# tlemane/kmtricks

Measured on AMD Instinct MI355X. Metric: k-mers merged/s (merge stage, sum over partitions of input records / time), higher is better.
Workload: dtype u64 keys / u32 counts (integer)

## Files before the change

### kmtricks_amd/csrc/kmx_api.hip

```cpp
#include "kmx_host.hpp"

#include <algorithm>
#include <chrono>
#include <cmath>
#include <sys/mman.h>
#include <unordered_map>
#include <mutex>
#include <cstdlib>
#include <cstring>
#include <memory>

using namespace kmx;

static thread_local std::string g_create_err;

void* kmx_ctx::dalloc(size_t bytes)
{
  if (bytes == 0) bytes = 256;
  if (bytes >= (8u << 20)) { size_t p2 = (size_t)1 << 23; while (p2 * 2 <= bytes) p2 *= 2; const size_t q = p2 >> 3; bytes = (bytes + q - 1) / q * q; }
  int best = -1;
  for (size_t i = 0; i < pool.size(); i++)
    if (!pool[i].used && pool[i].bytes >= bytes && pool[i].bytes <= 2 * bytes + (1u << 20) &&
        (best < 0 || pool[i].bytes < pool[best].bytes)) best = (int)i;
  if (best >= 0) { pool[best].used = true; return pool[best].p; }
// ... 511 lines not shown
    KMX_HIP(ctx, launch_merge_bf(mode == KMX_MODE_BFC, d_tasks, d_items, R->n_items, d_ticket, R->grid, R->bf_lds, ctx->stream));
  } else if (R->use_cols) {
    const TaskDev* d_subs = reinterpret_cast<const TaskDev*>(R->d_meta + R->o_subtasks);
    const uint2* d_subitems = reinterpret_cast<const uint2*>(R->d_meta + R->o_subitems);
    const ColsDev* d_cols = reinterpret_cast<const ColsDev*>(R->d_meta + R->o_cols);
    const uint2* d_citems = reinterpret_cast<const uint2*>(R->d_meta + R->o_citems);
    static const bool overlap = getenv("KMX_COLS_PREP_OVERLAP") != nullptr;
    hipStream_t ps = overlap ? ctx->aux : ctx->stream;
    if (!R->ev_pre) KMX_HIP(ctx, hipEventCreateWithFlags(&R->ev_pre, hipEventDisableTiming));
    if (overlap && ctx->stream_shared) {
      KMX_HIP(ctx, hipEventRecord(R->ev_pre, ctx->stream));
      KMX_HIP(ctx, hipStreamWaitEvent(ctx->aux, R->ev_pre, 0));
    }
    if (!overlap) KMX_HIP(ctx, hipStreamWaitEvent(ctx->stream, R->ev_up, 0));
    KMX_HIP(ctx, launch_range_bounds(kw, d_subs, nt, R->sub_max_n, R->sub_max_c, ps));
    KMX_HIP(ctx, CO.skel(d_subs, d_subitems, R->n_subitems, ps));
    KMX_HIP(ctx, CO.prep(d_tasks, d_subs, d_cols, nt, ps));
    {
      u32 max_slots = 0;
      for (auto& H : R->tasks) max_slots = std::max(max_slots, H.slots_cap);
      const char* const tenv = getenv("KMX_COLS_SEED_TRIES");
      KMX_HIP(ctx, CO.seeds(d_tasks, d_cols, nt, max_slots, tenv && atoi(tenv) > 0 ? (u32)atoi(tenv) : 0u, getenv("KMX_TRACE") != nullptr, ps));
    }
    KMX_HIP(ctx, hipEventRecord(R->ev_pre, ps));
    KMX_HIP(ctx, hipStreamWaitEvent(ctx->stream, R->ev_up, 0));
    KMX_HIP(ctx, launch_range_bounds(kw, d_tasks, nt, R->max_n, R->max_c, ctx->stream));
    KMX_HIP(ctx, hipStreamWaitEvent(ctx->stream, R->ev_pre, 0));
    if (R->ev0) KMX_HIP(ctx, hipEventRecord(R->ev0, ctx->stream));
    const u32 cols_grid_env = getenv("KMX_COLS_GRID") ? (u32)atoi(getenv("KMX_COLS_GRID")) : 0u;
    const u32 sparse_cus_env = getenv("KMX_SPARSE_CUS") ? (u32)atoi(getenv("KMX_SPARSE_CUS")) : 0u;
    KMX_HIP(ctx, CO.merge(mode, (R->cols_ext ? 1 : 0) | (R->cols_resc ? 2 : 0) | (R->cols_ord ? 4 : 0) | (R->cols_narrow ? 8 : 0), d_tasks, d_cols, d_citems, R->n_citems, d_ticket,
                          cols_grid_env ? std::min(cols_grid_env, R->cols_grid) : R->cols_grid, ctx->stream));
    if (R->ev0) { if (!R->ev_mid) KMX_HIP(ctx, hipEventCreate(&R->ev_mid)); KMX_HIP(ctx, hipEventRecord(R->ev_mid, ctx->stream)); }
    KMX_HIP(ctx, CO.sparse(mode | (R->cols_resc ? 2 : 0) | (R->cols_ord ? 4 : 0), d_tasks, d_cols, d_items, R->n_items, nt, d_ticket, sparse_cus_env ? std::min(sparse_cus_env, (u32)ctx->n_cu) : (u32)ctx->n_cu, ctx->stream));
    if (R->share_fix) {
      if ((size_t)R->max_n * 4 > 48 * 1024) KMX_HIP(ctx, hipFuncSetAttribute(reinterpret_cast<const void*>(&k_share_fix), hipFuncAttributeMaxDynamicSharedMemorySize, (int)std::min<size_t>((size_t)R->max_n * 4, 160 * 1024)));
      hipLaunchKernelGGL(k_share_fix, dim3((unsigned)ctx->n_cu * 2u, nt), dim3(256), (size_t)R->max_n * 4, ctx->stream, (const TaskDev*)d_tasks, kw);
      KMX_HIP(ctx, hipGetLastError());
    }
    if (R->ev0) KMX_HIP(ctx, hipEventRecord(R->ev1, ctx->stream));
    return mirror_and_mark(R);
  } else {
    if (with_bounds) KMX_HIP(ctx, launch_range_bounds(kw, d_tasks, nt, R->max_n, R->max_c, ctx->stream));
    if (R->ev0) KMX_HIP(ctx, hipEventRecord(R->ev0, ctx->stream));
    if (R->use_pivot) KMX_HIP(ctx, launch_merge_pivot(kw, mode, d_tasks, d_items, R->n_items, d_ticket, R->grid, ctx->stream));
    else if (R->rows_small) KMX_HIP(ctx, launch_merge_rows_s(kw, mode, d_tasks, d_items, R->n_items, d_ticket, R->grid, R->max_n, ctx->stream));
    else KMX_HIP(ctx, launch_merge_rows(kw, mode, d_tasks, d_items, R->n_items, d_ticket, R->grid, R->max_n, ctx->stream));
  }
  if (R->ev0) KMX_HIP(ctx, hipEventRecord(R->ev1, ctx->stream));
  return mirror_and_mark(R);
}

__global__ __launch_bounds__(256)
void k_share_fix(const TaskDev* __restrict__ tasks, u32 kw)
{
  extern __shared__ u32 sm_s[];
  const TaskDev& T = tasks[blockIdx.y];
  if (T.mode != KMX_MODE_COUNT || T.share_min <= max(1u, T.rec_min)) return;
  if (T.ctrl[2] & (u64)(ERR_FALLBACK | ERR_ROWS_OVERFLOW)) return;
  const u64 rows = T.ctrl[0];
  const u32 lane = threadIdx.x & 63u, N = T.N;
  for (u32 l = threadIdx.x; l < N; l += 256) sm_s[l] = T.soft_min[l];
  __syncthreads();
  const u64 nw = (u64)gridDim.x * 4u;
  for (u64 r = (u64)blockIdx.x * 4u + (threadIdx.x >> 6); r < rows; r += nw) {
    u32* const cnt = reinterpret_cast<u32*>(T.out + r * T.row_bytes + 8u * kw);
    u32 solid = 0, weak = 0;
// ... 1490 lines not shown
```

### kmtricks_amd/csrc/merge_cols.hip

```cpp
#include "kmx_host.hpp"
#include <algorithm>
#include <cstdio>
#include <cstring>

#ifndef KMX_CL_KW
#define KMX_CL_KW 1
#endif
#if KMX_CL_KW == 1
#define CLNS cols_k1
#elif KMX_CL_KW == 2
#define CLNS cols_k2
#elif KMX_CL_KW == 3
#define CLNS cols_k3
#else
#define CLNS cols_k4
#endif

namespace kmx { namespace CLNS {

#ifndef KMX_CL_TPB
#define KMX_CL_TPB 1024
#endif
constexpr int CL_TPB = KMX_CL_TPB;
constexpr int CL_WGS = 1024 / CL_TPB;
// ... 747 lines not shown
          rlo = (u32)rs; rhi = (u32)(rs >> 32);
          rn += __shfl_xor(rn, off);
        }
        if (on && r == 0 && rn) { atomicAdd(&T.stats[1 * (u64)N + li], (u64)rn); atomicAdd(&T.stats[5 * (u64)N + li], rs); }
      }
    }
    if (failed) atomicOr(&T.ctrl[2], (u64)ERR_FALLBACK);
    int t0 = tid; asm volatile("" : "+v"(t0));
    for (int t = t0; t < CL_NT * CL_PT; t += CL_TPB) ptab[t].idx = 0;
    __syncthreads();
  }
}

#ifndef KMX_CK_TPB0
#define KMX_CK_TPB0 256
#endif
#ifndef KMX_CK_TPB1
#define KMX_CK_TPB1 512
#endif
#ifndef KMX_CK_Z
#define KMX_CK_Z 16
#endif
#ifndef KMX_CK_OCC1
#define KMX_CK_OCC1 4
#endif
template <int MODE> __host__ __device__ constexpr int ck_tpb() { return MODE == 0 ? KMX_CK_TPB0 : KMX_CK_TPB1; }
constexpr int CK_Z = KMX_CK_Z;
#ifndef KMX_CK_SPEC2
#define KMX_CK_SPEC2 (KW == 1 ? 7 : 4)
#endif
constexpr int CK_SPEC4 = KW == 1 ? 5 : 4;
constexpr int CK_SPEC2 = KMX_CK_SPEC2;
constexpr int CK_CAND = 2048;
constexpr int CK_B2 = 1 << 15;
constexpr int CK_NPASS = 8;
constexpr int CK_UNI = CK_BITS / 8 + CK_B2 / 8;

struct SpDir { u32 base, n, dense_first, dense_n; };

__device__ __forceinline__ bool ck_less(CKey ka, u64 pa, CKey kb, u64 pb) { return !ck_eq(ka, kb) ? ck_lt(ka, kb) : pa < pb; }

__device__ __forceinline__ CKey ck_shfl_xor(CKey k, int m)
{
#if KMX_CL_KW == 1
  return (u64)__shfl_xor((unsigned long long)k, m);
#else
  CKey r; r.lo = (u64)__shfl_xor((unsigned long long)k.lo, m); r.hi = (u64)__shfl_xor((unsigned long long)k.hi, m); return r;
#endif
}
__device__ __forceinline__ void ck_chunk_steps(CKey (&k)[2], u64 (&p)[2], u32 base, u32 lane, u32 k2, u32 jtop)
{
  if (jtop >= 64u) {
    const bool asc = ((base + lane) & k2) == 0;
    if (ck_less(k[1], p[1], k[0], p[0]) == asc) { const CKey tk = k[0]; k[0] = k[1]; k[1] = tk; const u64 tp = p[0]; p[0] = p[1]; p[1] = tp; }
    jtop = 32;
  }
  for (u32 j = jtop; j > 0; j >>= 1) {
#pragma unroll
    for (int x = 0; x < 2; x++) {
      const CKey ok = ck_shfl_xor(k[x], (int)j); const u64 op = (u64)__shfl_xor((unsigned long long)p[x], (int)j);
      const bool asc = ((base + 64u * x + lane) & k2) == 0;
      const bool keep_min = ((lane & j) == 0) == asc;
      const bool other_less = ck_less(ok, op, k[x], p[x]);
      if (other_less == keep_min) { k[x] = ok; p[x] = op; }
    }
  }
// ... 42 lines not shown
  if (lane == 0) __hip_atomic_store(&chain[g], (1ULL << 62) | mine, __ATOMIC_RELAXED, __HIP_MEMORY_SCOPE_AGENT);
  u64 excl = 0;
  u32 i = g;
  for (;;) {
    const u64 v = lane < i ? __hip_atomic_load(&chain[i - 1 - lane], __ATOMIC_RELAXED, __HIP_MEMORY_SCOPE_AGENT) : (2ULL << 62);
    const u32 st = (u32)(v >> 62);
    const u64 inv = __ballot(st == 0), pfx = __ballot(st == 2);
    const u32 lim = inv ? (u32)__builtin_ctzll(inv) : 64u;
    const u64 pm = lim == 64u ? pfx : (pfx & ((1ULL << lim) - 1ULL));
    const u32 take = pm ? (u32)__builtin_ctzll(pm) + 1u : lim;
    u64 s = lane < take ? (v & VAL) : 0ULL;
#pragma unroll
    for (int off = 32; off > 0; off >>= 1) s += shfl_xor_u64(s, off);
    excl += s;
    if (pm) break;
    i -= take;
    if (take == 0) {
      __builtin_amdgcn_s_sleep(8);
      if (++spins > CK_LB_SPINS) {
        if (lane == 0) {
          atomicOr(err, (u64)ERR_FALLBACK);
          __threadfence();
          __hip_atomic_store(&chain[g], 2ULL << 62, __ATOMIC_RELAXED, __HIP_MEMORY_SCOPE_AGENT);
          atomicAdd(&kmx_cols_dbg[8], 1u); kmx_cols_dbg[10] = g; kmx_cols_dbg[11] = i;
        }
        return ~0ULL;
      }
    }
  }
  if (lane == 0) __hip_atomic_store(&chain[g], (2ULL << 62) | (excl + mine), __ATOMIC_RELAXED, __HIP_MEMORY_SCOPE_AGENT);
  return excl;
}

template <int MODE, bool RESC, bool ORD>
__global__ __launch_bounds__(ck_tpb<MODE>(), MODE == 1 ? KMX_CK_OCC1 : ORD ? 2 : 3)
void k_cols_sparse(const TaskDev* __restrict__ tasks, const ColsDev* __restrict__ cols, const uint2* __restrict__ items, u32 n_items, u32 n_tasks, u32* tkt)
{
  constexpr int CK_TPB = ck_tpb<MODE>();
  constexpr u32 CK_TS = CK_TPB >= 512 ? 4 : 2;
  constexpr int CK_SPEC = CK_TS == 4 ? CK_SPEC4 : CK_SPEC2;
  constexpr int CK_PTM = CK_CAND / CK_TPB;
  constexpr int CK_STAGE = CK_UNI / (CK_TPB / 64);
  __shared__ __attribute__((aligned(16))) u32 uni[CK_UNI / 4];
  u32* const bits = uni;
  u32* const bits2 = uni + CK_BITS / 32;
  __shared__ CKey ck[CK_CAND];
  __shared__ u64 cp[CK_CAND];
  __shared__ u32 runs[CK_CAND];
  __shared__ u32 wsum[CK_TPB / 64];
  __shared__ u32 total, ncand, rowbase, sover;
  __shared__ CKey dkeys[ORD ? 64 : 1];
  __shared__ u32 dpos[ORD ? 64 : 1];
  __shared__ u32 s_tk;
  __shared__ u64 s_base;
  u32* const parow = uni;
  static_assert((CK_TPB / 16) * 136 * 4 <= CK_UNI, "the lane groups' rows fit the block");
  auto ent_key = [](const u64* kp, u32 e) -> CKey {
#if KMX_CL_KW == 1
    return kp[EW * e];
#else
    CKey k; k.lo = kp[EW * e]; k.hi = kp[EW * e + 1]; return k;
#endif
  };
#ifdef KMX_PHASE_PROF
  long long spt[8] = {0, 0, 0, 0, 0, 0, 0, 0}; long long spc = clock64();
#define SPPH(i) do { const long long n_ = clock64(); spt[i] += n_ - spc; spc = n_; } while (0)
#else
#define SPPH(i) do {} while (0)
#endif
  const u32 tid = threadIdx.x, lane = tid & 63, wave = tid >> 6;
  auto pl_list = [](u64 pl) -> u32 { return (u32)(pl >> 32) & 0x7FFFFFFFu; };
  auto pl_solid = [](u64 pl) -> bool { return !RESC || !(pl & CL_NONSOLID); };
  if (tid == 0) { total = 0; sover = 0; }
  __syncthreads();

  auto group = [&](const TaskDev& T, const ColsDev& C, const u32 range, const u32 q, const u32 s_lo, const u32 s_hi, const u32 gord) -> bool {
    const u32 thr = RESC ? T.rec_min : max(1u, T.rec_min), share = RESC ? T.share_min : 0u, rt = C.rt, nsl = C.nblk * CL_NW, row_bytes = T.row_bytes;
    const u32 slot0 = (s_lo / rt + range) * CL_HALVES;
    SpDir* const dir = reinterpret_cast<SpDir*>(C.spdir);
    const bool single = nsl <= (u32)CK_TPB / CK_TS;
    const u64 sbase = (u64)(slot0 + q) * nsl;
// ... 3 lines not shown
    const u32 t0 = s_lo + tq * rt, te = min(s_hi, t0 + rt);
    u32 d0 = t0, dn = te - t0;
    if (CL_HALVES > 1) { const u32 mid = min(te, t0 + 56u); d0 = hq ? mid : t0; dn = hq ? te - mid : mid - t0; }
    if (s_hi == s_lo) { d0 = s_lo; dn = 0; }
    if (ORD && tid < dn) dkeys[tid] = reinterpret_cast<const CKey*>(C.skel)[d0 + tid];
    u32 n0 = 0; CKey kk0[CK_SPEC]; u64 pp0[CK_SPEC];
    const u64* kp0 = C.ovkeys; const u64* kpx0 = C.ovx;
    if (single) {
      const u32 sl = tid / CK_TS, sub = tid % CK_TS;
      const bool ok = sl < nsl;
      const uint2 ce = ok ? reinterpret_cast<const uint2*>(C.ovcnt)[sbase + sl] : make_uint2(0u, 0u);
      const u32 nraw = ce.x, xb = ce.y;
      kpx0 = C.ovx + (u64)(xb ? xb - 1u : 0u) * EW;
      const u32 lim0 = xb ? (u32)(CL_OVW + CL_XS) : (u32)CL_OVW;
      kp0 = C.ovkeys + (sbase + (ok ? sl : 0u)) * CL_OVW * EW;
#pragma unroll
      for (int x = 0; x < CK_SPEC; x++) { kk0[x] = ent_key(kp0, sub + CK_TS * x); pp0[x] = kp0[EW * (sub + CK_TS * x) + KW]; }
      n0 = min(nraw, lim0);
      if (nraw > lim0) sover = 1;
      if (sub == 0 && nraw) atomicAdd(&total, nraw);
    } else {
      for (u32 sl = tid; sl < nsl; sl += CK_TPB) {
        const uint2 ce = reinterpret_cast<const uint2*>(C.ovcnt)[sbase + sl];
        const u32 nraw = ce.x;
        if (nraw > (ce.y ? (u32)(CL_OVW + CL_XS) : (u32)CL_OVW)) sover = 1;
        if (nraw) atomicAdd(&total, nraw);
      }
    }
    __syncthreads();
    const u32 tot = total;
    const bool over = sover != 0;
    __syncthreads();
    SPPH(0);
    if (tid == 0) { total = 0; sover = 0; if (!ORD) { dir[(u64)gid * CK_NPASS].dense_first = d0; dir[(u64)gid * CK_NPASS].dense_n = dn; } }
    bool failed = false;
    if (over) { hand_back(1); if (!ORD) return false; failed = true; }
    if (!ORD && tot == 0) return true;
#ifndef KMX_CK_PER1
#define KMX_CK_PER1 1400
#endif
    const u32 per = (thr <= 1 ? (u32)KMX_CK_PER1 : 3000u) * (u32)CK_CAND / 2048u;
    u32 npass = 1;
    if (!(MODE == 1 && thr <= 1 && tot <= (u32)CK_CAND)) while (npass < (u32)CK_NPASS && tot > per * npass) npass <<= 1;
    if (!ORD && tot > per * npass * 2) { hand_back(3); return false; }
    if (ORD) {
      if (thr <= 1 && tot <= (u32)CK_CAND) npass = 1;
      while (npass > 1 && npass > dn) npass >>= 1;
    }
    auto each = [&](auto&& in_pass, auto&& f) {
      if (single) {
        const u32 sub = tid % CK_TS;
#pragma unroll
        for (int x = 0; x < CK_SPEC; x++)
          if (sub + CK_TS * x < n0 && in_pass(kk0[x])) f(kk0[x], pp0[x]);
        for (u32 e = sub + CK_TS * CK_SPEC; e < n0; e += CK_TS) {
          const u64* const kp = e < (u32)CL_OVW ? kp0 : kpx0; const u32 ee = e < (u32)CL_OVW ? e : e - (u32)CL_OVW;
          const CKey k = ent_key(kp, ee);
          if (!in_pass(k)) continue;
          f(k, kp[EW * ee + KW]);
        }
        return;
      }
      for (u32 sl0 = 0; sl0 < nsl; sl0 += CK_TPB / 4) {
        const u32 sl = sl0 + (tid >> 2), sub = tid & 3u;
        if (sl >= nsl) continue;
        const uint2 ce = reinterpret_cast<const uint2*>(C.ovcnt)[sbase + sl];
        const u32 xb = ce.y;
        const u32 n = min(ce.x, xb ? (u32)(CL_OVW + CL_XS) : (u32)CL_OVW);
        const u64* const kpb = C.ovkeys + (sbase + sl) * CL_OVW * EW;
        const u64* const kpx = C.ovx + (u64)(xb ? xb - 1u : 0u) * EW;
        for (u32 e = sub; e < n; e += 4) {
          const u64* const kp = e < (u32)CL_OVW ? kpb : kpx; const u32 ee = e < (u32)CL_OVW ? e : e - (u32)CL_OVW;
          const CKey k = ent_key(kp, ee);
          if (!in_pass(k)) continue;
          f(k, kp[EW * ee + KW]);
        }
      }
    };
    auto push = [&](CKey k, u64 pl) {
      const u64 act = __ballot(1);
      const u32 ldr = (u32)__builtin_ctzll(act);
      u32 b0 = 0;
      if (lane == ldr) b0 = atomicAdd(&ncand, (u32)__popcll(act));
      b0 = (u32)__shfl((int)b0, (int)ldr);
      const u32 ps = b0 + (u32)__popcll(act & ((1ULL << lane) - 1ULL));
      if (ps < (u32)CK_CAND) { ck[ps] = k; cp[ps] = pl; }
    };

    auto sort_pass = [&](const u32 pass, const bool final, const u32 dlo, const u32 dnp) -> u32 {
      constexpr bool BY_INTERVAL = MODE == 1;
      CKey plo = ck_inf(), phi = ck_inf(); bool has_lo = false, has_hi = false;
      if (ORD && npass > 1) { has_lo = pass > 0; has_hi = pass + 1 < npass; if (has_lo) plo = dkeys[dlo]; if (has_hi) phi = dkeys[dlo + dnp]; }
      auto in_pass = [&](CKey k) -> bool {
        if (npass <= 1) return true;
        if (ORD) return !(has_lo && ck_lt(k, plo)) && !(has_hi && !ck_lt(k, phi));
        return ((cl_mix(k) >> 24) & (npass - 1)) == pass;
      };
      if (thr > 1) {
        for (u32 t = tid; t < (u32)CK_BITS / 128; t += CK_TPB) reinterpret_cast<uint4*>(bits)[t] = make_uint4(0, 0, 0, 0);
        for (u32 t = tid; t < (u32)CK_B2 / 128; t += CK_TPB) reinterpret_cast<uint4*>(bits2)[t] = make_uint4(0, 0, 0, 0);
      } else {
        for (u32 t = tid; t < 512u; t += CK_TPB) bits[t] = 0;
      }
      if (tid == 0) ncand = 0;
      __syncthreads();
      SPPH(1);
      bool sorted = false;
      u32 nc1 = 0;
      if (thr <= 1 && !BY_INTERVAL) {
        each(in_pass, push);
        __syncthreads();
      }
      if (thr <= 1 && BY_INTERVAL) {
        constexpr u32 NS = 256, NIV = 320;
        u32* const ioff = bits;
        CKey* const sk = reinterpret_cast<CKey*>(bits + 1024);
        u64* const sp = reinterpret_cast<u64*>(bits + 1024 + NS * (sizeof(CKey) / 4));
        each(in_pass, push);
        __syncthreads();
        SPPH(7);
        nc1 = ncand;
        if (nc1 <= (u32)CK_CAND) {
          constexpr int PER = CK_CAND / CK_TPB;
          const u32 stride = (nc1 + NS - 1) / NS, ns = stride ? (nc1 + stride - 1) / stride : 0u, SP = ns <= 128u ? 128u : 256u;
          for (u32 t = tid; t < SP; t += CK_TPB) { sk[t] = t < ns ? ck[t * stride] : ck_inf(); sp[t] = t < ns ? cp[t * stride] : ~0ULL; }
          __syncthreads();
          ck_sort_block<CK_TPB>(sk, sp, SP, tid);
          CKey mk[PER]; u64 mp[PER]; u32 mb[PER], mo[PER];
#pragma unroll
          for (int x = 0; x < PER; x++) {
            const u32 i = tid + (u32)x * CK_TPB;
            mk[x] = ck_inf(); mp[x] = 0; mb[x] = 0xFFFFFFFFu; mo[x] = 0;
            if (i < nc1) { mk[x] = ck[i]; mp[x] = cp[i]; }
          }
          {
            u32 lo[PER], hi[PER];
#pragma unroll
            for (int x = 0; x < PER; x++) { lo[x] = 0; hi[x] = ns; }
#pragma unroll
            for (int it = 0; it < 9; it++) {
#pragma unroll
              for (int x = 0; x < PER; x++) {
                const u32 m = (lo[x] + hi[x]) >> 1;
                const bool open = lo[x] < hi[x];
                const bool below = open && ck_less(sk[min(m, NS - 1u)], sp[min(m, NS - 1u)], mk[x], mp[x]);
                lo[x] = below ? m + 1 : lo[x];
                hi[x] = (open && !below) ? m : hi[x];
              }
            }
#pragma unroll
            for (int x = 0; x < PER; x++) if (tid + (u32)x * CK_TPB < nc1) { mb[x] = lo[x]; mo[x] = atomicAdd(&ioff[lo[x]], 1u); }
          }
          __syncthreads();
          if (tid < 64) {
            u32 v[5]; u32 sum = 0;
#pragma unroll
// ... 16 lines not shown
            if (mb[x] != 0xFFFFFFFFu) {
              const u32 lo = ioff[mb[x]], hi = ioff[mb[x] + 1];
              u32 rr = lo;
              for (u32 j = lo; j < hi; j++) rr += ck_less(ck[j], cp[j], mk[x], mp[x]) ? 1u : 0u;
              mr[x] = rr;
            }
          }
          __syncthreads();
#pragma unroll
          for (int x = 0; x < PER; x++) if (mr[x] != 0xFFFFFFFFu) { ck[mr[x]] = mk[x]; cp[mr[x]] = mp[x]; }
          sorted = true;
        }
        __syncthreads();
      }
      if (thr > 1) {
        each(in_pass, [&](CKey k, u64) {
          const u32 hx = cl_mix(k);
          const u32 bit = hx & (CK_BITS - 1);
          const u32 old = atomicOr(&bits[bit >> 5], 1u << (bit & 31u));
          if ((old >> (bit & 31u)) & 1u) { const u32 b2 = (hx >> 7) & (CK_B2 - 1); atomicOr(&bits2[b2 >> 5], 1u << (b2 & 31u)); }
        });
        __syncthreads();
        SPPH(2);
      }
      if (thr > 1) {
        each(in_pass, [&](CKey k, u64 pl) {
          const u32 b2 = (cl_mix(k) >> 7) & (CK_B2 - 1); if (!((bits2[b2 >> 5] >> (b2 & 31u)) & 1u)) return;
          push(k, pl);
        });
        __syncthreads();
      }
      SPPH(3);
      const u32 nc = ncand;
      if (nc > (u32)CK_CAND) return CK_OVF;
      if (nc == 0) return 0u;
      if (!sorted) {
        u32 P = 128; while (P < nc) P <<= 1;
        for (u32 t = nc + tid; t < P; t += CK_TPB) { ck[t] = ck_inf(); cp[t] = ~0ULL; }
        __syncthreads();
        ck_sort_block<CK_TPB>(ck, cp, P, tid);
      }
      SPPH(4);
      u32 mine = 0, km = 0, rl[CK_PTM];
      const u32 pt = (nc + CK_TPB - 1) / CK_TPB;
#pragma unroll
      for (u32 x = 0; x < (u32)CK_PTM; x++) {
        rl[x] = 0;
        const u32 i = tid * pt + x;
        if (x < pt && i < nc) {
          const CKey k = ck[i];
          const bool first = i == 0 || !ck_eq(ck[i - 1], k);
          bool kept = first && (thr == 0 || (i + thr - 1 < nc && ck_eq(ck[i + thr - 1], k) && pl_solid(cp[i + thr - 1])));
          u32 len = 1;
          if (RESC && first) {
            while (i + len < nc && ck_eq(ck[i + len], k)) len++;
            u32 ns = 0; while (ns < len && pl_solid(cp[i + ns])) ns++;
            if (final && share && ns >= share) for (u32 e = ns; e < len; e++) { const u64 pl = cp[i + e]; atomicAdd(&T.stats[1 * (u64)T.N + pl_list(pl)], 1ULL); atomicAdd(&T.stats[5 * (u64)T.N + pl_list(pl)], (u64)(u32)pl); }
            if (final && kept && !(share && ns >= share)) for (u32 e = ns; e < len; e++) cp[i + e] &= ~0xFFFFFFFFULL;
          } else if (kept) { while (i + len < nc && ck_eq(ck[i + len], k)) len++; }
          if (kept) {
            rl[x] = i | (len << 11);
            if (ORD) {
              u32 lo = 0, hi = dnp;
              while (lo < hi) { const u32 m = (lo + hi) >> 1; if (ck_lt(dkeys[dlo + m], k)) lo = m + 1; else hi = m; }
              rl[x] |= lo << 24;
            }
          }
// ... 171 lines not shown
                if ((n8 & 1u) && sl == 0) reinterpret_cast<u64*>(row)[n8 - 1] = word(n8 - 1);
              } else {
                u32* const r4 = reinterpret_cast<u32*>(row);
                for (u32 t = sl; t < row_bytes / 4; t += SG) r4[t] = t < 2u * KW ? kword(t) : (t - 2u * KW == li ? cnt : 0u);
              }
            } else {
              put_bytes(row, [&](u32 w) -> u32 { return w < 2u * KW ? kword(w) : (w - 2u * KW == (li >> 5) ? bitv << (li & 31u) : 0u); });
            }
            continue;
          }
          if (MODE == 0) {
            if ((row_bytes & 7u) == 0) {
              auto word = [&](u32 t) -> u64 { return t < (u32)KW ? ((u64)kword(2 * t) | ((u64)kword(2 * t + 1) << 32)) : 0ULL; };
              const u32 n8 = row_bytes / 8, n16 = n8 >> 1;
              for (u32 t = sl; t < n16; t += SG) { u64x2 v; v.x = word(2 * t); v.y = word(2 * t + 1); *reinterpret_cast<u64x2*>(row + 16u * t) = v; }
              if ((n8 & 1u) && sl == 0) reinterpret_cast<u64*>(row)[n8 - 1] = word(n8 - 1);
            } else {
              u32* const r4 = reinterpret_cast<u32*>(row);
              for (u32 t = sl; t < row_bytes / 4; t += SG) r4[t] = t < 2u * KW ? kword(t) : 0u;
            }
            __builtin_amdgcn_fence(__ATOMIC_RELEASE, "wavefront");
            for (u32 e = sl; e < len; e += SG) { const u64 pl = cp[i0 + e]; reinterpret_cast<u32*>(row + KW * 8)[pl_list(pl)] = (u32)pl; }
          } else {
            u32* const pr = parow + sg * (SG == 8u ? 40u : 136u);
            const u32 nby = row_bytes - KW * 8, nw = (nby + 3) / 4;
            for (u32 t = sl; t < nw + 2 * KW + 1; t += SG) pr[t] = t < 2u * KW ? kword(t) : 0u;
            __builtin_amdgcn_fence(__ATOMIC_RELEASE, "wavefront");
            for (u32 e = sl; e < len; e += SG) { const u64 pl = cp[i0 + e]; const u32 li = pl_list(pl); if (!RESC || (u32)pl) atomicOr(&pr[2 * KW + (li >> 5)], 1u << (li & 31u)); }
            __builtin_amdgcn_fence(__ATOMIC_RELEASE, "wavefront");
            put_bytes(row, [&](u32 w) -> u32 { return pr[w]; });
          }
        }
        };
        if (ORD && MODE == 0 && (row_bytes & 7u) == 0 && row_bytes / 8 <= 512u) {
          constexpr int RF = 4;
          const u32 n8 = row_bytes / 8;
          const u32 rounds = max(1u, (dnp + (CK_TPB / 64) * RF - 1) / ((CK_TPB / 64) * RF));
          if (C.dnarrow) {
            const u8* const nar = C.dnarrow; const u32 npitch = C.npitch, nbs = C.nb, NL = T.N, FO = npitch - 16u;
            const u32 ng = (NL + 15u) / 16u;
            const u32 l0 = min(16u * lane, NL - 1u), fsh = 8u * (l0 / nbs);
            const u32 nval = lane < ng ? min(16u, NL - 16u * lane) : 0u;
            for (u32 c = 0; c < rounds; c++) {
              const u32 i0 = c * (CK_TPB / 64) * RF + wave * RF;
              uint4 nv[RF]; u64 fl[RF];
#pragma unroll
              for (int r = 0; r < RF; r++) {
                const u32 i = i0 + r;
                const u8* const nrow = nar + (u64)(d0 + dlo + (i < dnp ? i : 0)) * npitch;
                fl[r] = i < dnp ? *reinterpret_cast<const u64*>(nrow + FO) : 0ULL;
                nv[r] = (i < dnp && lane < ng) ? *reinterpret_cast<const uint4*>(nrow + 16u * lane) : make_uint4(0, 0, 0, 0);
              }
              sparse_rows((u32)(((u64)nk * c) / rounds), (u32)(((u64)nk * (c + 1)) / rounds));
#pragma unroll
              for (int r = 0; r < RF; r++) {
                const u32 i = i0 + r;
                if (i >= dnp) continue;
                u8* const row = T.out + (rb + dpos[i]) * row_bytes;
                if (lane == 0) {
                  u32 kw4[4] = {0, 0, 0, 0};
                  ck_store(kw4, dkeys[dlo + i]);
#pragma unroll
                  for (u32 d = 0; d < 2u * KW; d++) reinterpret_cast<u32*>(row)[d] = kw4[d];
                }
                if (nval == 0) continue;
                u8* const out = row + 8u * KW + 64u * lane;
                const u32 by[4] = {nv[r].x, nv[r].y, nv[r].z, nv[r].w};
                const bool flagged = ((fl[r] >> fsh) & 0xFFULL) != 0;
                if (!flagged) {
#pragma unroll
                  for (u32 q4 = 0; q4 < 4; q4++) {
                    const u32 b = by[q4];
                    if (4 * q4 + 4 <= nval) { u64x2 v; v.x = (u64)(b & 0xFFu) | ((u64)((b >> 8) & 0xFFu) << 32); v.y = (u64)((b >> 16) & 0xFFu) | ((u64)(b >> 24) << 32); *reinterpret_cast<u64x2*>(out + 16u * q4) = v; }
                    else if (4 * q4 + 2 <= nval) *reinterpret_cast<u64*>(out + 16u * q4) = (u64)(b & 0xFFu) | ((u64)((b >> 8) & 0xFFu) << 32);
                  }
                } else {
                  const u32* const wsrc = dense_src(i); u32* const cnt = reinterpret_cast<u32*>(row + 8u * KW);
                  for (u32 l = 0; l < nval; l++) { const u32 b = (by[l >> 2] >> (8u * (l & 3u))) & 0xFFu; cnt[16u * lane + l] = b == 255u ? wsrc[16u * lane + l] : b; }
                }
              }
            }
          } else
          for (u32 c = 0; c < rounds; c++) {
            const u32 i0 = c * (CK_TPB / 64) * RF + wave * RF;
            u64 w[RF][8];
#pragma unroll
            for (int r = 0; r < RF; r++) {
              const u32 i = i0 + r;
              const u64* const s8 = reinterpret_cast<const u64*>(dense_src(i < dnp ? i : 0));
              u32 kw4[4] = {0, 0, 0, 0};
              ck_store(kw4, dkeys[dlo + (i < dnp ? i : 0)]);
#pragma unroll
              for (int x = 0; x < 8; x++) {
                const u32 t = 64 * x + lane;
                w[r][x] = 0;
                if (i < dnp && t < n8) w[r][x] = t < (u32)KW ? ((u64)kw4[2 * (t & 1u)] | ((u64)kw4[2 * (t & 1u) + 1] << 32)) : s8[t - KW];
              }
            }
            sparse_rows((u32)(((u64)nk * c) / rounds), (u32)(((u64)nk * (c + 1)) / rounds));
#pragma unroll
            for (int r = 0; r < RF; r++) {
// ... 20 lines not shown
        const u32 nk = sort_pass(pass, true, 0, 0);
        if (nk == CK_OVF) { hand_back(3); return false; }
        if (tid == 0) { dir[(u64)gid * CK_NPASS + pass].base = 0; dir[(u64)gid * CK_NPASS + pass].n = 0; }
        if (nk == 0) { __syncthreads(); continue; }
        if (tid == 0) {
          const u64 at = atomicAdd(&T.ctrl[0], (u64)nk);
          atomicAdd(&T.ctrl[3], (u64)nk); atomicAdd(&T.ctrl[6], (u64)nk);
          if (at + nk > T.out_cap_rows) { atomicOr(&T.ctrl[2], (u64)ERR_ROWS_OVERFLOW); rowbase = 0xFFFFFFFFu; }
          else { rowbase = (u32)at; dir[(u64)gid * CK_NPASS + pass].base = (u32)at; dir[(u64)gid * CK_NPASS + pass].n = nk; }
        }
        __syncthreads();
        const u32 rb = rowbase;
        SPPH(5);
        if (rb != 0xFFFFFFFFu) write_pass((u64)rb, nk, 0, 0, false);
        else __syncthreads();
      }
      return true;
    }
    __syncthreads();
    u32 nks = 0;
    while (!failed && tot) {
      bool ovf = false;
      nks = 0;
      if (npass == 1) { const u32 r = sort_pass(0, true, 0, dn); if (r == CK_OVF) ovf = true; else nks = r; __syncthreads(); }
      else for (u32 p = 0; p < npass; p++) {
        const u32 dlo = (u32)(((u64)dn * p) / npass), dhi = (u32)(((u64)dn * (p + 1)) / npass);
        const u32 r = sort_pass(p, false, dlo, dhi - dlo);
        __syncthreads();
        if (r == CK_OVF) { ovf = true; break; }
        nks += r;
      }
      if (!ovf) break;
      if (npass * 2 > (u32)CK_NPASS || npass * 2 > dn) { hand_back(3); failed = true; break; }
      npass *= 2;
    }
    const u64 grows = failed ? 0ULL : (u64)dn + nks;
    if (wave == 0) { const u64 b = ck_lookback(C.chain, gord, grows, lane, &T.ctrl[2]); if (lane == 0) s_base = b; }
    else if (npass == 1 && !failed && tid - 64u < dn) dense_places(tid - 64u, nks, 0, dn);
    __syncthreads();
    SPPH(5);
    if (failed) return false;
    if (s_base == ~0ULL) { hand_back(12); return false; }
    auto count_rows = [&]() { if (tid == 0 && nks) { atomicAdd(&T.ctrl[0], (u64)nks); atomicAdd(&T.ctrl[3], (u64)nks); atomicAdd(&T.ctrl[6], (u64)nks); } };
    const u64 base = s_base;
    if (base + grows > T.out_cap_rows) { if (tid == 0) atomicOr(&T.ctrl[2], (u64)ERR_ROWS_OVERFLOW); count_rows(); return true; }
    if (npass == 1) write_pass(base, nks, 0, dn, true);
    else {
      u64 b = base;
      for (u32 p = 0; p < npass; p++) {
        const u32 dlo = (u32)(((u64)dn * p) / npass), dhi = (u32)(((u64)dn * (p + 1)) / npass);
        const u32 nk = sort_pass(p, true, dlo, dhi - dlo);
        __syncthreads();
        write_pass(b, nk, dlo, dhi - dlo, false);
        b += nk + (dhi - dlo);
      }
    }
    count_rows();
    return true;
  };

  if (!ORD) {
    const u32 item = blockIdx.x;
    if (item < n_items) {
      const TaskDev& T = tasks[items[item].x];
      const ColsDev& C = cols[items[item].x];
      if (!__syncthreads_or((__hip_atomic_load(&T.ctrl[2], __ATOMIC_RELAXED, __HIP_MEMORY_SCOPE_AGENT) & (u64)(ERR_FALLBACK | ERR_ROWS_OVERFLOW)) != 0)) {
// ... 95 lines not shown
  u8* const dst0 = body + goff[blockIdx.x] * row_bytes;
  __shared__ u32 rnk[GA_KEYS];
  auto rank_of = [&](u32 i) -> u32 {
    const CKey k = key_at(i);
    u32 rank = 0;
    for (int l = 0; l <= CK_NPASS; l++) {
      u32 a = lo[l], b = lo[l + 1];
      if (i >= a && i < b) { rank += i - a; continue; }
      while (a < b) { const u32 m = (a + b) >> 1; if (ck_lt(key_at(m), k)) a = m + 1; else b = m; }
      rank += a - lo[l];
    }
    return rank;
  };
  for (u32 i = tid; i < min(n, (u32)GA_KEYS); i += GA_TPB) rnk[i] = rank_of(i);
  __syncthreads();
  for (u32 i = wave; i < n; i += GA_TPB / 64) {
    const u32 rank = i < (u32)GA_KEYS ? rnk[i] : rank_of(i);
    const u8* s = src_row(i);
    u8* d = dst0 + (u64)rank * row_bytes;
    if ((row_bytes & 7u) == 0) {
      const u32 n8 = row_bytes / 8;
      for (u32 t0 = 0; t0 < n8; t0 += 512) {
        u64 w[8];
#pragma unroll
        for (int x = 0; x < 8; x++) { const u32 t = t0 + 64 * x + lane; w[x] = t < n8 ? reinterpret_cast<const u64*>(s)[t] : 0ULL; }
#pragma unroll
        for (int x = 0; x < 8; x++) { const u32 t = t0 + 64 * x + lane; if (t < n8) reinterpret_cast<u64*>(d)[t] = w[x]; }
      }
    } else if ((row_bytes & 3u) == 0) for (u32 t = lane; t < row_bytes / 4; t += 64) reinterpret_cast<u32*>(d)[t] = reinterpret_cast<const u32*>(s)[t];
    else for (u32 t = lane; t < row_bytes; t += 64) d[t] = s[t];
  }
}

void cols_dbg_dump()
{
  u32 h[16];
  if (hipMemcpyFromSymbol(h, HIP_SYMBOL(kmx_cols_dbg), sizeof(h)) != hipSuccess) return;
  if (h[9]) fprintf(stderr, "[kmx merge] k_cols_sparse: the group count of the batch was beyond every task's room (%u workgroups stopped at the room)\n", h[9]);
  if (h[8]) fprintf(stderr, "[kmx merge] k_cols_sparse: %u look-backs given up (last: group %u, %u entries still unpublished in front of it)\n", h[8], h[10], h[11]);
  fprintf(stderr, "[kmx merge] k_merge_cols hand-back reasons: no collision-free row table %u, slice overflow %u (wave-tiles; largest %u, in a range's last tile %u, first tile %u), kept key outside the row keys %u, check table full %u, lists too divergent %u (tasks)\n", h[0], h[1], h[5], h[6], h[7], h[2], h[3], h[4]);
  memset(h, 0, sizeof(h)); (void)hipMemcpyToSymbol(HIP_SYMBOL(kmx_cols_dbg), h, sizeof(h));
}
void cols_seeds_dump()
{
  u32 h[12];
  if (hipMemcpyFromSymbol(h, HIP_SYMBOL(kmx_cols_tries), sizeof(h)) != hipSuccess) return;
  u64 n = 0; for (int i = 0; i < 10; i++) n += h[i];
  if (n + h[11] == 0) return;
  fprintf(stderr, "[kmx merge] k_cols_seeds: hash words tried per tile: 1: %u, 2: %u, 3-4: %u, 5-8: %u, 9-16: %u, 17-32: %u, 33-64: %u, 65-128: %u, more: %u; tiles without row keys %u, most tries %u, none found %u\n",
          h[0], h[1], h[2], h[3], h[4], h[5], h[6], h[7], h[8], h[9], h[10], h[11]);
  memset(h, 0, sizeof(h)); (void)hipMemcpyToSymbol(HIP_SYMBOL(kmx_cols_tries), h, sizeof(h));
}
#ifdef KMX_PHASE_PROF
void cols_phase_prof_dump()
{
  u64 h[8];
  if (hipMemcpyFromSymbol(h, HIP_SYMBOL(kmx_cols_prof), sizeof(h)) != hipSuccess) return;
  u64 tot = 0; for (int i = 0; i < 8; i++) tot += h[i];
  static const char* nm[8] = {"item setup", "window wait", "scan", "bar(scan)", "tile out", "bar(out)", "-", "-"};
  for (int i = 0; i < 6; i++) fprintf(stderr, "[cols] %-12s %6.2f%%  %llu\n", nm[i], tot ? 100.0 * h[i] / tot : 0.0, h[i]);
  memset(h, 0, sizeof(h));
  (void)hipMemcpyToSymbol(HIP_SYMBOL(kmx_cols_prof), h, sizeof(h));
  if (hipMemcpyFromSymbol(h, HIP_SYMBOL(kmx_sparse_prof), sizeof(h)) != hipSuccess) return;
  tot = 0; for (int i = 0; i < 8; i++) tot += h[i];
  static const char* sn[8] = {"group entries", "zero maps", "mark twice | sample + place", "candidates | rank", "sort", "runs + claim", "rows", "gather (rec-min 1)"};
  for (int i = 0; i < 8; i++) fprintf(stderr, "[sparse] %-14s %6.2f%%  %llu\n", sn[i], tot ? 100.0 * h[i] / tot : 0.0, h[i]);
  memset(h, 0, sizeof(h));
  (void)hipMemcpyToSymbol(HIP_SYMBOL(kmx_sparse_prof), h, sizeof(h));
}
#endif

int cols_lds_bytes() { return CL_IMG + CL_NT * CL_PT * (int)sizeof(ClEnt) + 64 + 256; }
u32 cols_halves() { return CL_HALVES; }
u32 cols_wgs_per_cu() { return CL_WGS; }
u32 cols_block_lists() { return CL_NB; }
u32 cols_tile_rows(u32 nb) { return std::max(1u, std::min<u32>((u32)CL_RT, (u32)CL_IMG / (4u * std::max(1u, nb)))); }
u64 cols_scratch_keys(u32 slots, u32 nblk) { return (u64)slots * CL_HALVES * nblk * CL_NW * CL_OVW * EW; }
// ... 7 lines not shown
  return hipGetLastError();
}
hipError_t launch_cols_prep(const TaskDev* tasks, const TaskDev* subs, const ColsDev* cols, u32 n_tasks, hipStream_t st)
{
  hipLaunchKernelGGL(k_cols_prep, dim3(n_tasks), dim3(CP_TPB), 0, st, tasks, subs, cols);
  return hipGetLastError();
}
hipError_t launch_cols_seeds(const TaskDev* tasks, const ColsDev* cols, u32 n_tasks, u32 max_slots, u32 max_tries, bool trace, hipStream_t st)
{
  const u32 per = (u32)(CS_TPB / 64);
  hipLaunchKernelGGL(k_cols_seeds, dim3((max_slots + per - 1) / per, n_tasks), dim3(CS_TPB), 0, st, tasks, cols, max_tries ? max_tries : CS_TRIES, trace ? 1u : 0u);
  return hipGetLastError();
}
template <int MODE, bool EXT, bool RESC, bool ORD, bool NAR>
static hipError_t launch_merge_cols_as(const TaskDev* tasks, const ColsDev* cols, const uint2* items, u32 n_items, u32* ticket, u32 grid_x, hipStream_t st)
{
  const int lds = cols_lds_bytes();
  hipError_t e = hipFuncSetAttribute(reinterpret_cast<const void*>(&k_merge_cols<MODE, EXT, RESC, ORD, NAR>), hipFuncAttributeMaxDynamicSharedMemorySize, lds);
  if (e != hipSuccess) return e;
  hipLaunchKernelGGL((k_merge_cols<MODE, EXT, RESC, ORD, NAR>), dim3(grid_x), dim3(CL_TPB), lds, st, tasks, cols, items, n_items, ticket);
  return hipGetLastError();
}
hipError_t launch_merge_cols(int mode, int ext, const TaskDev* tasks, const ColsDev* cols, const uint2* items, u32 n_items, u32* ticket, u32 grid_x, hipStream_t st)
{
  const bool x = ext & 1, r = (ext & 2) != 0, o = (ext & 4) != 0, n = (ext & 8) != 0 && o && mode == 0;
#define KMX_CL_L3(M, X, R) (o ? launch_merge_cols_as<M, X, R, true, false>(tasks, cols, items, n_items, ticket, grid_x, st) : launch_merge_cols_as<M, X, R, false, false>(tasks, cols, items, n_items, ticket, grid_x, st))
#define KMX_CL_LAUNCH(M) (r ? (x ? KMX_CL_L3(M, true, true) : KMX_CL_L3(M, false, true)) : (x ? KMX_CL_L3(M, true, false) : KMX_CL_L3(M, false, false)))
  if (n) return r ? (x ? launch_merge_cols_as<0, true, true, true, true>(tasks, cols, items, n_items, ticket, grid_x, st) : launch_merge_cols_as<0, false, true, true, true>(tasks, cols, items, n_items, ticket, grid_x, st))
                  : (x ? launch_merge_cols_as<0, true, false, true, true>(tasks, cols, items, n_items, ticket, grid_x, st) : launch_merge_cols_as<0, false, false, true, true>(tasks, cols, items, n_items, ticket, grid_x, st));
  return mode == 0 ? KMX_CL_LAUNCH(0) : KMX_CL_LAUNCH(1);
#undef KMX_CL_L3
#undef KMX_CL_LAUNCH
}
template <int MODE, bool RESC>
static hipError_t launch_cols_sparse_ord(const TaskDev* tasks, const ColsDev* cols, u32 n_tasks, u32* ticket, u32 n_cu, hipStream_t st)
{
  static int per_cu = 0;
  if (per_cu == 0) {
    int n = 0;
    if (hipOccupancyMaxActiveBlocksPerMultiprocessor(&n, reinterpret_cast<const void*>(&k_cols_sparse<MODE, RESC, true>), ck_tpb<MODE>(), 0) != hipSuccess || n < 1) { (void)hipGetLastError(); n = 1; }
    per_cu = n;
  }
  hipLaunchKernelGGL((k_cols_sparse<MODE, RESC, true>), dim3(n_cu * (u32)per_cu), dim3(ck_tpb<MODE>()), 0, st, tasks, cols, (const uint2*)nullptr, 0u, n_tasks, ticket);
  return hipGetLastError();
}
hipError_t launch_cols_sparse(int mode, const TaskDev* tasks, const ColsDev* cols, const uint2* range_items, u32 n_items, u32 n_tasks, u32* ticket, u32 n_cu, hipStream_t st)
{
  if (mode & 4) {
    switch (mode & 3) {
      case 0: return launch_cols_sparse_ord<0, false>(tasks, cols, n_tasks, ticket, n_cu, st);
      case 1: return launch_cols_sparse_ord<1, false>(tasks, cols, n_tasks, ticket, n_cu, st);
      case 2: return launch_cols_sparse_ord<0, true>(tasks, cols, n_tasks, ticket, n_cu, st);
      default: return launch_cols_sparse_ord<1, true>(tasks, cols, n_tasks, ticket, n_cu, st);
    }
  }
  const dim3 grid(n_items, CK_Z), block(ck_tpb<0>()), block1(ck_tpb<1>());
  switch (mode & 3) {
    case 0: hipLaunchKernelGGL((k_cols_sparse<0, false, false>), grid, block, 0, st, tasks, cols, range_items, n_items, n_tasks, ticket); break;
    case 1: hipLaunchKernelGGL((k_cols_sparse<1, false, false>), grid, block1, 0, st, tasks, cols, range_items, n_items, n_tasks, ticket); break;
    case 2: hipLaunchKernelGGL((k_cols_sparse<0, true, false>), grid, block, 0, st, tasks, cols, range_items, n_items, n_tasks, ticket); break;
    default: hipLaunchKernelGGL((k_cols_sparse<1, true, false>), grid, block1, 0, st, tasks, cols, range_items, n_items, n_tasks, ticket); break;
  }
  return hipGetLastError();
}
u64 cols_dir_bytes(u32 slots) { return (u64)slots * CL_HALVES * CK_NPASS * sizeof(SpDir); }
u32 cols_groups(u32 slots) { return slots * CL_HALVES; }
hipError_t launch_cols_offsets(const ColsDev* cols, u32 task, u64* goff, hipStream_t st)
{
  hipLaunchKernelGGL(k_cols_offsets, dim3(1), dim3(1024), 0, st, cols, task, goff);
  return hipGetLastError();
}
hipError_t launch_cols_gather(const TaskDev* tasks, const ColsDev* cols, u32 task, u32 n_groups, const u64* goff, u8* body, hipStream_t st)
{
  hipLaunchKernelGGL(k_cols_gather<true>, dim3(n_groups), dim3(GA_TPB), 0, st, tasks, cols, task, goff, body);
  return hipGetLastError();
}
hipError_t launch_cols_order(const TaskDev* tasks, const ColsDev* cols, u32 task, u32 n_groups, const u64* goff, u32* order, hipStream_t st)
{
  hipLaunchKernelGGL(k_cols_gather<false>, dim3(n_groups), dim3(GA_TPB), 0, st, tasks, cols, task, goff, reinterpret_cast<u8*>(order));
  return hipGetLastError();
}

static const ColsOps g_ops = {cols_lds_bytes, cols_block_lists, cols_wgs_per_cu, cols_tile_rows, cols_scratch_keys, cols_scratch_counts, cols_ext_entries, cols_skel_cap,
                              launch_cols_skel, launch_cols_prep, launch_cols_seeds, launch_merge_cols, launch_cols_sparse, cols_dir_bytes, cols_groups, launch_cols_offsets,
                              launch_cols_gather, launch_cols_order, cols_dbg_dump, cols_seeds_dump,
// ... 18 lines not shown
```

Baseline: 134.2 billion.

## Specialize sparse column kernel for narrow byte-wide store with smaller candidate buffers

Adds a NAR template variant of the file-order sparse count kernel, selected when the narrow side store is in use. It halves the shared candidate arrays, reads a single flag byte per row instead of a u64 word, and exposes occupancy, speculation depth and row-unroll as macros. Smaller LDS use is meant to let more workgroups fit per CU. The cost is more candidate overflows, each of which forces an extra finer pass. Debug counters for those retries are also added.

```diff
diff --git a/kmtricks_amd/csrc/kmx_api.hip b/kmtricks_amd/csrc/kmx_api.hip
--- a/kmtricks_amd/csrc/kmx_api.hip
+++ b/kmtricks_amd/csrc/kmx_api.hip
@@ -567,7 +567,7 @@
     KMX_HIP(ctx, CO.merge(mode, (R->cols_ext ? 1 : 0) | (R->cols_resc ? 2 : 0) | (R->cols_ord ? 4 : 0) | (R->cols_narrow ? 8 : 0), d_tasks, d_cols, d_citems, R->n_citems, d_ticket,
                           cols_grid_env ? std::min(cols_grid_env, R->cols_grid) : R->cols_grid, ctx->stream));
     if (R->ev0) { if (!R->ev_mid) KMX_HIP(ctx, hipEventCreate(&R->ev_mid)); KMX_HIP(ctx, hipEventRecord(R->ev_mid, ctx->stream)); }
-    KMX_HIP(ctx, CO.sparse(mode | (R->cols_resc ? 2 : 0) | (R->cols_ord ? 4 : 0), d_tasks, d_cols, d_items, R->n_items, nt, d_ticket, sparse_cus_env ? std::min(sparse_cus_env, (u32)ctx->n_cu) : (u32)ctx->n_cu, ctx->stream));
+    KMX_HIP(ctx, CO.sparse(mode | (R->cols_resc ? 2 : 0) | (R->cols_ord ? 4 : 0) | (R->cols_narrow ? 8 : 0), d_tasks, d_cols, d_items, R->n_items, nt, d_ticket, sparse_cus_env ? std::min(sparse_cus_env, (u32)ctx->n_cu) : (u32)ctx->n_cu, ctx->stream));
     if (R->share_fix) {
       if ((size_t)R->max_n * 4 > 48 * 1024) KMX_HIP(ctx, hipFuncSetAttribute(reinterpret_cast<const void*>(&k_share_fix), hipFuncAttributeMaxDynamicSharedMemorySize, (int)std::min<size_t>((size_t)R->max_n * 4, 160 * 1024)));
       hipLaunchKernelGGL(k_share_fix, dim3((unsigned)ctx->n_cu * 2u, nt), dim3(256), (size_t)R->max_n * 4, ctx->stream, (const TaskDev*)d_tasks, kw);
diff --git a/kmtricks_amd/csrc/merge_cols.hip b/kmtricks_amd/csrc/merge_cols.hip
--- a/kmtricks_amd/csrc/merge_cols.hip
+++ b/kmtricks_amd/csrc/merge_cols.hip
@@ -803,6 +803,22 @@
 constexpr int CK_SPEC4 = KW == 1 ? 5 : 4;
 constexpr int CK_SPEC2 = KMX_CK_SPEC2;
 constexpr int CK_CAND = 2048;
+#ifndef KMX_CK_OCC0N
+#define KMX_CK_OCC0N 2
+#endif
+#ifndef KMX_CK_SPEC2N
+#define KMX_CK_SPEC2N (KMX_CK_OCC0N >= 3 ? 4 : CK_SPEC2)
+#endif
+#ifndef KMX_CK_SPEC2NR
+#define KMX_CK_SPEC2NR (KMX_CK_OCC0N >= 3 ? 3 : CK_SPEC2)
+#endif
+#ifndef KMX_CK_RFN
+#define KMX_CK_RFN (KMX_CK_OCC0N >= 3 ? 3 : 4)
+#endif
+#ifndef KMX_CK_CAND_NAR
+#define KMX_CK_CAND_NAR 1024
+#endif
+constexpr int CK_CAND_NAR = KMX_CK_CAND_NAR;
 constexpr int CK_B2 = 1 << 15;
 constexpr int CK_NPASS = 8;
 constexpr int CK_UNI = CK_BITS / 8 + CK_B2 / 8;
@@ -911,21 +927,23 @@
   return excl;
 }
 
-template <int MODE, bool RESC, bool ORD>
-__global__ __launch_bounds__(ck_tpb<MODE>(), MODE == 1 ? KMX_CK_OCC1 : ORD ? 2 : 3)
+template <int MODE, bool RESC, bool ORD, bool NAR = false>
+__global__ __launch_bounds__(ck_tpb<MODE>(), MODE == 1 ? KMX_CK_OCC1 : ORD ? (NAR ? KMX_CK_OCC0N : 2) : 3)
 void k_cols_sparse(const TaskDev* __restrict__ tasks, const ColsDev* __restrict__ cols, const uint2* __restrict__ items, u32 n_items, u32 n_tasks, u32* tkt)
 {
   constexpr int CK_TPB = ck_tpb<MODE>();
   constexpr u32 CK_TS = CK_TPB >= 512 ? 4 : 2;
-  constexpr int CK_SPEC = CK_TS == 4 ? CK_SPEC4 : CK_SPEC2;
-  constexpr int CK_PTM = CK_CAND / CK_TPB;
+  static_assert(!NAR || (MODE == 0 && ORD), "the byte-wide side store is the file-order count build's");
+  constexpr int CAND = NAR ? CK_CAND_NAR : CK_CAND;
+  constexpr int CK_SPEC = CK_TS == 4 ? CK_SPEC4 : NAR ? (RESC ? KMX_CK_SPEC2NR : KMX_CK_SPEC2N) : CK_SPEC2;
+  constexpr int CK_PTM = CAND / CK_TPB;
   constexpr int CK_STAGE = CK_UNI / (CK_TPB / 64);
   __shared__ __attribute__((aligned(16))) u32 uni[CK_UNI / 4];
   u32* const bits = uni;
   u32* const bits2 = uni + CK_BITS / 32;
-  __shared__ CKey ck[CK_CAND];
-  __shared__ u64 cp[CK_CAND];
-  __shared__ u32 runs[CK_CAND];
+  __shared__ CKey ck[CAND];
+  __shared__ u64 cp[CAND];
+  __shared__ u32 runs[CAND];
   __shared__ u32 wsum[CK_TPB / 64];
   __shared__ u32 total, ncand, rowbase, sover;
   __shared__ CKey dkeys[ORD ? 64 : 1];
@@ -995,19 +1013,19 @@
     const bool over = sover != 0;
     __syncthreads();
     SPPH(0);
-    if (tid == 0) { total = 0; sover = 0; if (!ORD) { dir[(u64)gid * CK_NPASS].dense_first = d0; dir[(u64)gid * CK_NPASS].dense_n = dn; } }
+    if (tid == 0) { total = 0; sover = 0; if (NAR && tot) atomicAdd(&kmx_cols_dbg[14], 1u); if (!ORD) { dir[(u64)gid * CK_NPASS].dense_first = d0; dir[(u64)gid * CK_NPASS].dense_n = dn; } }
     bool failed = false;
     if (over) { hand_back(1); if (!ORD) return false; failed = true; }
     if (!ORD && tot == 0) return true;
 #ifndef KMX_CK_PER1
 #define KMX_CK_PER1 1400
 #endif
-    const u32 per = (thr <= 1 ? (u32)KMX_CK_PER1 : 3000u) * (u32)CK_CAND / 2048u;
+    const u32 per = thr <= 1 ? (u32)KMX_CK_PER1 * (u32)CAND / 2048u : 3000u;
     u32 npass = 1;
-    if (!(MODE == 1 && thr <= 1 && tot <= (u32)CK_CAND)) while (npass < (u32)CK_NPASS && tot > per * npass) npass <<= 1;
+    if (!(MODE == 1 && thr <= 1 && tot <= (u32)CAND)) while (npass < (u32)CK_NPASS && tot > per * npass) npass <<= 1;
     if (!ORD && tot > per * npass * 2) { hand_back(3); return false; }
     if (ORD) {
-      if (thr <= 1 && tot <= (u32)CK_CAND) npass = 1;
+      if (thr <= 1 && tot <= (u32)CAND) npass = 1;
       while (npass > 1 && npass > dn) npass >>= 1;
     }
     auto each = [&](auto&& in_pass, auto&& f) {
@@ -1047,7 +1065,7 @@
       if (lane == ldr) b0 = atomicAdd(&ncand, (u32)__popcll(act));
       b0 = (u32)__shfl((int)b0, (int)ldr);
       const u32 ps = b0 + (u32)__popcll(act & ((1ULL << lane) - 1ULL));
-      if (ps < (u32)CK_CAND) { ck[ps] = k; cp[ps] = pl; }
+      if (ps < (u32)CAND) { ck[ps] = k; cp[ps] = pl; }
     };
 
     auto sort_pass = [&](const u32 pass, const bool final, const u32 dlo, const u32 dnp) -> u32 {
@@ -1083,8 +1101,8 @@
         __syncthreads();
         SPPH(7);
         nc1 = ncand;
-        if (nc1 <= (u32)CK_CAND) {
-          constexpr int PER = CK_CAND / CK_TPB;
+        if (nc1 <= (u32)CAND) {
+          constexpr int PER = CAND / CK_TPB;
           const u32 stride = (nc1 + NS - 1) / NS, ns = stride ? (nc1 + stride - 1) / stride : 0u, SP = ns <= 128u ? 128u : 256u;
           for (u32 t = tid; t < SP; t += CK_TPB) { sk[t] = t < ns ? ck[t * stride] : ck_inf(); sp[t] = t < ns ? cp[t * stride] : ~0ULL; }
           __syncthreads();
@@ -1167,7 +1185,7 @@
       }
       SPPH(3);
       const u32 nc = ncand;
-      if (nc > (u32)CK_CAND) return CK_OVF;
+      if (nc > (u32)CAND) return CK_OVF;
       if (nc == 0) return 0u;
       if (!sorted) {
         u32 P = 128; while (P < nc) P <<= 1;
@@ -1405,23 +1423,24 @@
           }
         }
         };
-        if (ORD && MODE == 0 && (row_bytes & 7u) == 0 && row_bytes / 8 <= 512u) {
-          constexpr int RF = 4;
+        if (NAR || (ORD && MODE == 0 && (row_bytes & 7u) == 0 && row_bytes / 8 <= 512u)) {
+          constexpr int RF = NAR ? KMX_CK_RFN : 4;
           const u32 n8 = row_bytes / 8;
           const u32 rounds = max(1u, (dnp + (CK_TPB / 64) * RF - 1) / ((CK_TPB / 64) * RF));
-          if (C.dnarrow) {
+          if (NAR || C.dnarrow) {
             const u8* const nar = C.dnarrow; const u32 npitch = C.npitch, nbs = C.nb, NL = T.N, FO = npitch - 16u;
             const u32 ng = (NL + 15u) / 16u;
-            const u32 l0 = min(16u * lane, NL - 1u), fsh = 8u * (l0 / nbs);
+            const u32 l0 = min(16u * lane, NL - 1u), fby = l0 / nbs, fsh = 8u * fby;
             const u32 nval = lane < ng ? min(16u, NL - 16u * lane) : 0u;
             for (u32 c = 0; c < rounds; c++) {
               const u32 i0 = c * (CK_TPB / 64) * RF + wave * RF;
-              uint4 nv[RF]; u64 fl[RF];
+              uint4 nv[RF]; typename std::conditional<NAR, u32, u64>::type fl[RF];
 #pragma unroll
               for (int r = 0; r < RF; r++) {
                 const u32 i = i0 + r;
                 const u8* const nrow = nar + (u64)(d0 + dlo + (i < dnp ? i : 0)) * npitch;
-                fl[r] = i < dnp ? *reinterpret_cast<const u64*>(nrow + FO) : 0ULL;
+                if (NAR) fl[r] = i < dnp ? (u32)nrow[FO + fby] : 0u;
+                else fl[r] = i < dnp ? *reinterpret_cast<const u64*>(nrow + FO) : 0ULL;
                 nv[r] = (i < dnp && lane < ng) ? *reinterpret_cast<const uint4*>(nrow + 16u * lane) : make_uint4(0, 0, 0, 0);
               }
               sparse_rows((u32)(((u64)nk * c) / rounds), (u32)(((u64)nk * (c + 1)) / rounds));
@@ -1439,7 +1458,7 @@
                 if (nval == 0) continue;
                 u8* const out = row + 8u * KW + 64u * lane;
                 const u32 by[4] = {nv[r].x, nv[r].y, nv[r].z, nv[r].w};
-                const bool flagged = ((fl[r] >> fsh) & 0xFFULL) != 0;
+                const bool flagged = NAR ? fl[r] != 0 : (((u64)fl[r] >> fsh) & 0xFFULL) != 0;
                 if (!flagged) {
 #pragma unroll
                   for (u32 q4 = 0; q4 < 4; q4++) {
@@ -1526,6 +1545,7 @@
       }
       if (!ovf) break;
       if (npass * 2 > (u32)CK_NPASS || npass * 2 > dn) { hand_back(3); failed = true; break; }
+      if (tid == 0) atomicAdd(&kmx_cols_dbg[13], 1u);
       npass *= 2;
     }
     const u64 grows = failed ? 0ULL : (u64)dn + nks;
@@ -1687,8 +1707,17 @@
   }
 }
 
+static void cols_retries_dump()
+{
+  u32 h[2];
+  if (hipMemcpyFromSymbol(h, HIP_SYMBOL(kmx_cols_dbg), sizeof(h), 13 * sizeof(u32)) != hipSuccess) return;
+  if (h[1]) fprintf(stderr, "[kmx merge] k_cols_sparse, byte-wide build: %u of %u slice groups cut finer after their candidates overflowed a pass\n", h[0], h[1]);
+  else if (h[0]) fprintf(stderr, "[kmx merge] k_cols_sparse: %u slice groups cut finer after their candidates overflowed a pass\n", h[0]);
+  if (h[0] | h[1]) { memset(h, 0, sizeof(h)); (void)hipMemcpyToSymbol(HIP_SYMBOL(kmx_cols_dbg), h, sizeof(h), 13 * sizeof(u32)); }
+}
 void cols_dbg_dump()
 {
+  cols_retries_dump();
   u32 h[16];
   if (hipMemcpyFromSymbol(h, HIP_SYMBOL(kmx_cols_dbg), sizeof(h)) != hipSuccess) return;
   if (h[9]) fprintf(stderr, "[kmx merge] k_cols_sparse: the group count of the batch was beyond every task's room (%u workgroups stopped at the room)\n", h[9]);
@@ -1698,6 +1727,7 @@
 }
 void cols_seeds_dump()
 {
+  cols_retries_dump();
   u32 h[12];
   if (hipMemcpyFromSymbol(h, HIP_SYMBOL(kmx_cols_tries), sizeof(h)) != hipSuccess) return;
   u64 n = 0; for (int i = 0; i < 10; i++) n += h[i];
@@ -1771,25 +1801,25 @@
 #undef KMX_CL_L3
 #undef KMX_CL_LAUNCH
 }
-template <int MODE, bool RESC>
+template <int MODE, bool RESC, bool NAR = false>
 static hipError_t launch_cols_sparse_ord(const TaskDev* tasks, const ColsDev* cols, u32 n_tasks, u32* ticket, u32 n_cu, hipStream_t st)
 {
   static int per_cu = 0;
   if (per_cu == 0) {
     int n = 0;
-    if (hipOccupancyMaxActiveBlocksPerMultiprocessor(&n, reinterpret_cast<const void*>(&k_cols_sparse<MODE, RESC, true>), ck_tpb<MODE>(), 0) != hipSuccess || n < 1) { (void)hipGetLastError(); n = 1; }
+    if (hipOccupancyMaxActiveBlocksPerMultiprocessor(&n, reinterpret_cast<const void*>(&k_cols_sparse<MODE, RESC, true, NAR>), ck_tpb<MODE>(), 0) != hipSuccess || n < 1) { (void)hipGetLastError(); n = 1; }
     per_cu = n;
   }
-  hipLaunchKernelGGL((k_cols_sparse<MODE, RESC, true>), dim3(n_cu * (u32)per_cu), dim3(ck_tpb<MODE>()), 0, st, tasks, cols, (const uint2*)nullptr, 0u, n_tasks, ticket);
+  hipLaunchKernelGGL((k_cols_sparse<MODE, RESC, true, NAR>), dim3(n_cu * (u32)per_cu), dim3(ck_tpb<MODE>()), 0, st, tasks, cols, (const uint2*)nullptr, 0u, n_tasks, ticket);
   return hipGetLastError();
 }
 hipError_t launch_cols_sparse(int mode, const TaskDev* tasks, const ColsDev* cols, const uint2* range_items, u32 n_items, u32 n_tasks, u32* ticket, u32 n_cu, hipStream_t st)
 {
   if (mode & 4) {
     switch (mode & 3) {
-      case 0: return launch_cols_sparse_ord<0, false>(tasks, cols, n_tasks, ticket, n_cu, st);
+      case 0: return (mode & 8) ? launch_cols_sparse_ord<0, false, true>(tasks, cols, n_tasks, ticket, n_cu, st) : launch_cols_sparse_ord<0, false>(tasks, cols, n_tasks, ticket, n_cu, st);
       case 1: return launch_cols_sparse_ord<1, false>(tasks, cols, n_tasks, ticket, n_cu, st);
-      case 2: return launch_cols_sparse_ord<0, true>(tasks, cols, n_tasks, ticket, n_cu, st);
+      case 2: return (mode & 8) ? launch_cols_sparse_ord<0, true, true>(tasks, cols, n_tasks, ticket, n_cu, st) : launch_cols_sparse_ord<0, true>(tasks, cols, n_tasks, ticket, n_cu, st);
       default: return launch_cols_sparse_ord<1, true>(tasks, cols, n_tasks, ticket, n_cu, st);
     }
   }
```

Result: no change. 133.3 billion (-0.7%).
